# Volxel/Volxel

Hardware: AMD Instinct MI355X
Metric: Gsamples/s raymarch @512^3 vol, 1080p; achieved HBM GB/s vs peak, 1/2/4/8 GPU (higher is better)
Workload: dtype f32

## Files before the change

### include/volxel_hip.h

```cpp
#ifndef VOLXEL_HIP_H
#define VOLXEL_HIP_H

#include <stdint.h>

#ifdef __cplusplus
extern "C" {
#endif

#define VX_OK 0
#define VX_ERR_INVALID 1
#define VX_ERR_DEVICE 2
#define VX_ERR_NO_VOLUME 3
#define VX_ERR_NO_DEVICE 4

enum VxRenderMode {
  VX_MODE_DEFAULT = 0,
  VX_MODE_NO_DDA = 1,
  VX_MODE_RAYMARCH = 2,
  VX_MODE_DVR = 3,
  VX_MODE_DVR_PHONG = 4,
  VX_MODE_MIP = 5,
  VX_MODE_MINIP = 6
};

// ... 356 lines not shown
  int32_t source;
  float iso;
  uint32_t box_lo[3];
  uint32_t box_hi[3];
  uint32_t max_vertices;
  uint32_t max_triangles;
} VxMeshParams;
typedef struct VxMeshResult {
  uint64_t vertices, triangles, active_blocks, blocks;
  uint32_t bbox_lo[3], bbox_hi[3];
} VxMeshResult;
int vx_mesh_extract(VxContext* ctx, const VxMeshParams* params, VxMeshResult* out);
int vx_mesh_read(VxContext* ctx, float* verts_xyz, int32_t* cells_xyz, uint32_t* tris);
int vx_mesh_stats(VxContext* ctx, uint32_t* launches, double* kernel_ms);

int vx_debug_unorm_table(VxContext* ctx, float* out256);
int vx_debug_build_skip_mask(const uint32_t* range_packed, const uint32_t brick_count[3], const float* tf_rgba,
                             uint32_t tf_len, const VxParams* params, uint32_t* bits_out, uint32_t* level_out,
                             uint32_t dims_out[3]);
int vx_debug_build_projection_bounds(const uint32_t* range_packed, const uint32_t brick_count[3], const VxParams* params,
                                     float* bounds_out, uint32_t* level_out, uint32_t dims_out[3]);
int vx_debug_classify_miss_blocks(const VxParams* params, uint32_t width, uint32_t height, uint8_t* flags_out, uint32_t* n_out);
int vx_debug_last_launch_blocks(VxContext* ctx, uint32_t* heavy_out, uint32_t* miss_out);

#ifdef __cplusplus
}
#endif
#endif
```

### volxel_amd/_abi.py

```python
from __future__ import annotations

import ctypes as C
import os
import re

_ROOT = os.path.dirname(os.path.dirname(os.path.abspath(__file__)))
INCLUDE_DIR = os.path.join(_ROOT, "include")
LIB_PATH = os.environ.get("VOLXEL_HIP_LIB") or os.path.join(os.path.dirname(os.path.abspath(__file__)), "libvolxel_hip.so")

_CTYPES = {
    "float": C.c_float, "double": C.c_double, "int32_t": C.c_int32, "uint32_t": C.c_uint32,
    "uint64_t": C.c_uint64, "int64_t": C.c_int64,
}


def struct_from_header(header: str, name: str):
    text = open(os.path.join(INCLUDE_DIR, header)).read()
    text = re.sub(r"/\*.*?\*/", "", text, flags=re.S)
    m = re.search(r"typedef\s+struct\s+%s\s*\{(.*?)\}\s*%s\s*;" % (name, name), text, flags=re.S)
    if not m:
        raise RuntimeError(f"struct {name} not found in {header}")
    fields = []
    for decl in m.group(1).split(";"):
        decl = decl.strip()
# ... 106 lines not shown
        "vx_read_accum": ([vp, vp], i32),
        "vx_read_display": ([vp, vp, C.c_float, C.c_float], i32),
        "vx_read_display_scaled": ([vp, vp, u32, u32, C.c_float, C.c_float], i32),
        "vx_slab_info": ([vp, P(u64), P(u32)], i32),
        "vx_probe_tile_costs": ([vp, vp, u32], i32),
        "vx_set_tile_order": ([vp, vp, u32], i32),
        "vx_render_size": ([vp, P(u32), P(u32)], i32),
        "vx_slab_device_ptr": ([vp, P(vp)], i32),
        "vx_detile": ([vp, vp, vp], i32),
        "vx_get_counters": ([vp, P(VxCounters)], i32),
        "vx_reset_counters": ([vp], i32),
        "vx_device_info": ([vp, C.c_char_p, u32, P(u32), P(u64)], i32),
        "vx_version": ([], C.c_char_p),
        "vx_debug_unorm_table": ([vp, vp], i32),
        "vx_debug_rng": ([vp, i32, vp, vp, u32, vp], i32),
        "vx_probe_gather_rate": ([vp, u32, u32, P(C.c_double), P(u32)], i32),
        "vx_probe_gather_spread": ([vp, u32, P(u64)], i32),
        "vx_probe_valu_rate": ([vp, P(C.c_double), P(u32)], i32),
        "vx_upload_stats": ([vp, P(C.c_double), P(u64), P(i32)], i32),
        "vx_debug_build_skip_mask": ([vp, P(u32), vp, u32, P(VxParams), vp, P(u32), P(u32)], i32),
        "vx_debug_build_projection_bounds": ([vp, P(u32), P(VxParams), vp, P(u32), P(u32)], i32),
        "vx_debug_classify_miss_blocks": ([P(VxParams), u32, u32, vp, P(u32)], i32),
        "vx_debug_last_launch_blocks": ([vp, P(u32), P(u32)], i32),
        "vx_shadow_stats": ([vp, P(u64), P(u64), P(C.c_double)], i32),
        "vx_debug_read_shadow_grid": ([vp, vp, P(u32)], i32),
        "vx_slice": ([vp, P(VxSliceParams), vp, vp], i32),
        "vx_slice_stats": ([vp, P(u64), P(C.c_double)], i32),
        "vx_isosurface": ([vp, P(VxIsoParams), vp, vp], i32),
        "vx_iso_stats": ([vp, P(u64), P(u64), P(u64), P(u64), P(u64), P(C.c_double)], i32),
        "vx_segment": ([vp, P(VxSegmentParams), P(VxSegmentResult)], i32),
        "vx_segment_read_mask": ([vp, vp, u64], i32),
        "vx_slice_segment_mask": ([vp, P(VxSliceParams), vp], i32),
        "vx_segment_stats": ([vp, P(u32), P(u64), P(C.c_double)], i32),
        "vx_set_segment_view": ([vp, i32], i32),
        "vx_get_segment_view": ([vp, P(i32)], i32),
        "vx_segment_edit": ([vp, P(VxSegmentEditParams), P(VxSegmentResult)], i32),
        "vx_segment_write_mask": ([vp, vp, u64, P(VxSegmentResult)], i32),
        "vx_segment_edit_stats": ([vp, P(u32), P(C.c_double)], i32),
        "vx_segment_threshold": ([vp, P(VxSegmentParams), P(VxSegmentResult)], i32),
        "vx_segment_islands": ([vp, P(VxIslandsParams), P(VxIslandsResult)], i32),
        "vx_islands_read": ([vp, u64, u64, P(VxIsland)], i32),
        "vx_islands_read_labels": ([vp, vp, u64], i32),
        "vx_islands_stats": ([vp, P(u32), P(C.c_double)], i32),
        "vx_segment_distance": ([vp, P(VxDistanceParams), P(VxDistanceResult)], i32),
        "vx_distance_read": ([vp, vp, u64], i32),
        "vx_segment_margin": ([vp, P(VxMarginParams), P(VxSegmentResult)], i32),
# ... 45 lines not shown
```

### volxel_amd/csrc/vx_api.hip

```cpp
#include <hip/hip_runtime.h>

#include <algorithm>
#include <cmath>
#include <cstdio>
#include <cstdlib>
#include <cstring>
#include <string>
#include <vector>

#include "vx_dvr.hpp"
#include "vx_dvr_lds.hpp"
#include "vx_dvr_miss.hpp"
#include "vx_kernels.hpp"
#include "vx_shadow.hpp"
#include "vx_projection.hpp"
#include "vx_context.hpp"

using namespace vx;

namespace {

thread_local std::string g_create_error;

bool dvr_miss_switch() {
  const char* v = getenv("VX_DVR_MISS");
  return !(v && atoi(v) == 0);
}
Switches read_switches() {
  Switches sw;
  if (const char* v = getenv("VX_DVR_KERNEL"); v && !strcmp(v, "generic")) sw.dvr_variant = 0;
  if (const char* v = getenv("VX_DVR_FUSE")) sw.dvr_fuse = atoi(v) != 0;
  if (const char* v = getenv("VX_RAY_SHORTCUTS"); v && atoi(v) == 0) sw.ray_shortcuts = false;
  if (const char* v = getenv("VX_AUTO_CELLQUAD_MAX_BYTES")) sw.cellquad_max_bytes = strtoull(v, nullptr, 10);
  if (const char* v = getenv("VX_SEG_CHECK_MAX")) sw.seg_check_max = (uint32_t)std::min(std::max(atoi(v), 1), 4096);
  if (const char* v = getenv("VX_DIST_LDS_BYTES")) sw.dist_lds_bytes = (uint32_t)std::min(std::max(atoi(v), 256), 65536);
  sw.dvr_miss = dvr_miss_switch();
  return sw;
}

static void drain_events(VxContext* c) {
  for (auto& e : c->pending_events) {
    (void)hipEventSynchronize(e.b);
    float ms = 0.f;
    if (hipEventElapsedTime(&ms, e.a, e.b) == hipSuccess) {
      if (e.merge) {
        c->merge_ms += ms;
      } else {
        c->kernel_ms += ms;
        c->last_kernel_ms = ms;
      }
    }
    e.merge = false;
    c->free_events.push_back(e);
  }
  c->pending_events.clear();
}

static void update_tilemap(VxContext* c) {
  TileMap& t = c->tm;
// ... 214 lines not shown

enum class Kernel {
  DVR_LDS,
  PROJ_LDS,
  DVR_CQ,
  GENERIC,
};
struct LaunchPlan {
  Kernel kernel = Kernel::GENERIC;
  int mode = VX_MODE_DVR;
  int layout = VX_LAYOUT_REFERENCE;
  bool phong = false;
  bool minip = false;
  bool shadow = false;
  bool skip = false;
  bool u8 = false;
  bool probe = false;
  ShadowGrid light{};
  const float* bounds = nullptr;
  const uint32_t* order = nullptr;
  dim3 grid, block{256};
  dim3 miss_grid{0};
  const uint32_t* miss_order = nullptr;
  size_t lds = 0;
  bool fuse = false;
  bool segv = false;
  const uint32_t* segm = nullptr;
  uint32_t seg_inv = 0u;
};

static bool tuned_possible(const VxContext* c) {
  return c->sw.dvr_variant != 0 && !c->params.debug_hits && c->tf_len <= TF_LDS_MAX &&
         (c->params.dvr_ert_tau > 0.0f || proj_mode(c->params.render_mode));
}
static bool use_lds_kernel(const VxContext* c) {
  if (!tuned_possible(c)) return false;
  if (proj_mode(c->params.render_mode))
    return eff_layout(c) == VX_LAYOUT_BRICKF32 || (eff_layout(c) == VX_LAYOUT_BRICKU8 && c->vol.dv.bu != nullptr);
  if (eff_layout(c) == VX_LAYOUT_BRICKU8)
    return (c->params.render_mode == VX_MODE_DVR || c->params.render_mode == VX_MODE_DVR_PHONG) && c->vol.dv.bu != nullptr;
  if (c->params.render_mode == VX_MODE_DVR) return eff_layout(c) == VX_LAYOUT_BRICKF32;
  return c->params.render_mode == VX_MODE_DVR_PHONG && c->vol.dv.bf != nullptr;
}
static bool is_tuned(const VxContext* c) {
  const bool dvr_cq = c->params.render_mode == VX_MODE_DVR && eff_layout(c) == VX_LAYOUT_CELLQUAD;
  return tuned_possible(c) && (dvr_cq || use_lds_kernel(c));
// ... 32 lines not shown
  if (lp.kernel == Kernel::PROJ_LDS) {
    lp.skip = p.dvr_skip_empty && c->proj_dev && !c->vol.proj_table.stale;
    lp.bounds = lp.skip ? c->proj_dev : nullptr;
  } else {
    lp.skip = p.dvr_skip_empty && c->vol.dv.skip_bits;
  }
  if (c->vol.seg_view != VX_SEGVIEW_OFF && lds_window_kernel(lp.kernel)) {
    lp.segv = true;
    lp.segm = reinterpret_cast<const uint32_t*>(c->vol.seg.seg);
    lp.seg_inv = c->vol.seg_view == VX_SEGVIEW_HIDE ? ~0u : 0u;
    lp.skip = false;
    lp.bounds = nullptr;
  }
  lp.u8 = lp.layout == VX_LAYOUT_BRICKU8 && c->vol.dv.bu;
  lp.probe = probe;
  lp.order = probe ? nullptr : c->order;
  const bool lds_window = lds_window_kernel(lp.kernel);
  lp.grid = dim3(frame_blocks(c) * (lds_window && mo.count == 0u ? 1u : mo.count));
  lp.fuse = c->sw.dvr_fuse && folds(lp.kernel, lp.mode, mo.count);
  lp.lds = lds_bytes(c, lp);
  const VxContext::MissSplit& ms = c->miss;
  if (lp.kernel == Kernel::DVR_LDS && !lp.phong && !lp.shadow && !lp.segv && mo.count > 1u && c->sw.dvr_miss && ms.proved > 0u &&
      ms.table.current(p) && ms.blocks == frame_blocks(c) && !ms.split_stale) {
    lp.grid = dim3((ms.blocks - ms.n_miss) * mo.count);
    lp.order = ms.order_heavy;
    lp.miss_grid = dim3(ms.n_miss * mo.count);
    lp.miss_order = ms.order_miss;
  }
  return lp;
}

template <class F>
static void with_mode(int m, F&& f) {
  switch (m) {
    case VX_MODE_DEFAULT: f(std::integral_constant<int, VX_MODE_DEFAULT>{}); break;
    case VX_MODE_NO_DDA: f(std::integral_constant<int, VX_MODE_NO_DDA>{}); break;
    case VX_MODE_RAYMARCH: f(std::integral_constant<int, VX_MODE_RAYMARCH>{}); break;
    case VX_MODE_DVR: f(std::integral_constant<int, VX_MODE_DVR>{}); break;
    case VX_MODE_MIP: f(std::integral_constant<int, VX_MODE_MIP>{}); break;
    case VX_MODE_MINIP: f(std::integral_constant<int, VX_MODE_MINIP>{}); break;
    default: f(std::integral_constant<int, VX_MODE_DVR_PHONG>{}); break;
  }
}

static int launch_planned(VxContext* c, const LaunchPlan& lp, const MultiOut& mo, float weight) {
  if (mo.fuse && !folds(lp.kernel, lp.mode, mo.count))
    VX_FAIL(c, VX_ERR_INVALID, "render launch: running mean to fold (MultiOut::fuse) for a kernel that does not fold it");
  const VxParams& p = c->params;
  const DevVolume& v = c->vol.dv;
  const TileMap& tm = c->tm;
  const float4* tf = c->tf;
  const uint32_t n = c->tf_len;
  const hipStream_t s = c->stream;
  switch (lp.kernel) {
    case Kernel::DVR_LDS:
      if (lp.segv) {
        with_bool(lp.u8, [&](auto u8) {
          with_bool(lp.phong, [&](auto ph) {
            constexpr bool PH = decltype(ph)::value;
            hipLaunchKernelGGL((render_dvr_lds_seg<(PH ? VX_LDS_S_PHONG : VX_LDS_S), PH, decltype(u8)::value>), lp.grid, lp.block,
                               lp.lds, s, p, v, tf, n, mo, weight, tm, lp.order, lp.segm, lp.seg_inv);
          });
        });
        break;
      }
      if (lp.miss_grid.x != 0u)
        hipLaunchKernelGGL(render_dvr_miss, lp.miss_grid, lp.block, mo.fuse ? 4u * 320u * sizeof(float) : 0u, s, p, v, tf, n, mo,
                           weight, tm, lp.miss_order);
      if (lp.grid.x == 0u) break;
      with_bool(lp.skip, [&](auto sk) {
        with_bool(lp.u8, [&](auto u8) {
          constexpr bool SK = decltype(sk)::value, U8 = decltype(u8)::value;
          if (lp.shadow) {
            hipLaunchKernelGGL((render_dvr_lds_shadow<VX_LDS_S, SK, U8>), lp.grid, lp.block, lp.lds, s, p, v, tf, n, mo, weight, tm,
                               lp.order, lp.light);
            return;
          }
          with_bool(lp.phong, [&](auto ph) {
            constexpr bool PH = decltype(ph)::value;
            hipLaunchKernelGGL((render_dvr_lds<(PH ? VX_LDS_S_PHONG : VX_LDS_S), PH, SK, U8>), lp.grid, lp.block, lp.lds, s, p, v, tf,
                               n, mo, weight, tm, lp.order);
          });
        });
      });
      break;
    case Kernel::PROJ_LDS:
      if (lp.segv) {
        with_bool(lp.minip, [&](auto mi) {
          with_bool(lp.u8, [&](auto u8) {
            hipLaunchKernelGGL((render_proj_lds_seg<VX_LDS_S, decltype(mi)::value, decltype(u8)::value>), lp.grid, lp.block, lp.lds, s,
                               p, v, tf, n, mo, weight, tm, lp.order, lp.segm, lp.seg_inv);
// ... 14 lines not shown
      with_bool(lp.skip, [&](auto sk) {
        with_bool(lp.probe, [&](auto pr) {
          hipLaunchKernelGGL((render_dvr_cq<4, decltype(sk)::value, decltype(pr)::value>), lp.grid, lp.block, lp.lds, s, p, v, tf, n,
                             mo, weight, tm, lp.order);
        });
      });
      break;
    default:
      with_layout(lp.layout, [&](auto lay) {
        constexpr int LAY = decltype(lay)::value;
        if (lp.shadow) {
          hipLaunchKernelGGL((render_generic_shadow<LAY>), lp.grid, lp.block, lp.lds, s, p, v, tf, n, mo, weight, tm, lp.light);
          return;
        }
        with_mode(lp.mode, [&](auto m) {
          hipLaunchKernelGGL((render_generic<decltype(m)::value, LAY>), lp.grid, lp.block, lp.lds, s, p, v, tf, n, mo, weight, tm);
        });
      });
  }
  VX_HIP(c, hipGetLastError());
  {
    const uint32_t slots = mo.count == 0u ? 1u : mo.count;
    c->miss.last_heavy = lp.grid.x / slots;
    c->miss.last_miss = lp.miss_grid.x / slots;
  }
  return VX_OK;
}

static int set_slab_table(VxContext* c, const std::vector<const float4*>& t) {
  if (t == c->slab_table_host) return VX_OK;
  c->slab_table_host.clear();
  VX_HIP(c, hipStreamSynchronize(c->stream));
  if (int rc = c->slab_table.ensure(c, t.size())) return rc;
  VX_HIP(c, hipMemcpy(c->slab_table, t.data(), t.size() * sizeof(float4*), hipMemcpyHostToDevice));
  c->slab_table_host = t;
  return VX_OK;
}

static int launch_detile(VxContext* c, float4* image) {
  if (c->slab_table_host.size() != c->tm.shard_count)
    VX_FAIL(c, VX_ERR_INVALID, "detile: %zu slabs for %u shards", c->slab_table_host.size(), c->tm.shard_count);
  dim3 grid((c->W + 15) / 16, (c->H + 15) / 16);
  hipLaunchKernelGGL(detile, grid, dim3(256), 0, c->stream, (const float4* const*)c->slab_table, image, c->tm);
  VX_HIP(c, hipGetLastError());
  return VX_OK;
}

// ... 15 lines not shown
    if (m->W != d->W || m->H != d->H || m->tm.shard_count != t.size())
      VX_FAIL(c, VX_ERR_INVALID, "member %zu (device %d): framebuffer differs from member 0's", i, m->device);
    t[i] = m->slab;
  }
  VX_HIP(c, hipSetDevice(d->device));
  if (int rc = set_slab_table(d, t)) return member_fail(c, 0, rc);
  for (size_t i = 1; i < t.size(); ++i) {
    VxContext* m = c->members[i];
    VX_HIP(c, hipSetDevice(m->device));
    VX_HIP(c, hipEventRecord(m->done, m->stream));
  }
  VX_HIP(c, hipSetDevice(d->device));
  for (size_t i = 1; i < t.size(); ++i) VX_HIP(c, hipStreamWaitEvent(d->stream, c->members[i]->done, 0));
  return on_member0(c, launch_detile(d, d->image));
}

static int ensure_miss_split(VxContext* c) {
  VxContext::MissSplit& ms = c->miss;
  const VxParams& p = c->params;
  if (!c->sw.dvr_miss || p.render_mode != VX_MODE_DVR || !use_lds_kernel(c)) return VX_OK;
  const uint32_t nb = frame_blocks(c);
  if (!ms.table.current(p) || ms.blocks != nb) {
    ms.table.stale = true;
    std::vector<uint8_t> img;
    ms.proved = ms.n_miss = 0;
    ms.blocks = nb;
    if (classify_miss_blocks(p, c->W, c->H, img) != 0u) {
      const TileMap& tm = c->tm;
      const uint32_t nbx = (c->W + 15u) / 16u;
      auto morton_x = [](uint32_t m) { return (m & 1u) | ((m >> 1) & 2u) | ((m >> 2) & 4u); };
      ms.flags_host.assign(nb, 0);
      for (uint32_t b = 0; b < nb; ++b) {
        const uint32_t lt = (b >> 7) * 8u + (b & 7u), wt = ((b >> 3) & 15u) * 4u;
        const uint32_t pos = lt * tm.shard_count + tm.shard_rank;
        const uint32_t t = (!c->tile_perm_host.empty() && pos < tm.n_tiles) ? c->tile_perm_host[pos] : pos;
        const uint32_t x0 = (t % tm.tiles_x) * 64u + morton_x(wt) * 8u, y0 = (t / tm.tiles_x) * 64u + morton_x(wt >> 1) * 8u;
        if (lt >= tm.tiles_per_shard || t >= tm.n_tiles || x0 >= tm.W || y0 >= tm.H) {
          ms.flags_host[b] = 1;
        } else if (img[(size_t)(y0 >> 4) * nbx + (x0 >> 4)]) {
          ms.flags_host[b] = 1;
          ms.proved += 1;
        }
        ms.n_miss += ms.flags_host[b];
      }
    }
    if (ms.proved > 0u) {
      if (ms.flags.cap < nb || ms.order_heavy.cap < nb || ms.order_miss.cap < nb) {
        VX_HIP(c, hipStreamSynchronize(c->stream));
        if (int rc = ms.flags.alloc(c, nb)) return rc;
        if (int rc = ms.order_heavy.alloc(c, nb)) return rc;
        if (int rc = ms.order_miss.alloc(c, nb)) return rc;
      }
      VxContext::MissSplit::Stage& st = ms.stage[ms.next_stage];
      ms.next_stage ^= 1;
      if (st.pending) VX_HIP(c, hipEventSynchronize(st.done));
      st.pending = false;
      if (st.cap < nb) {
        if (st.p) (void)hipHostFree(st.p);
        st.p = nullptr;
        st.cap = 0;
        VX_HIP(c, hipHostMalloc(reinterpret_cast<void**>(&st.p), nb, hipHostMallocDefault));
        st.cap = nb;
      }
      if (!st.done) VX_HIP(c, hipEventCreateWithFlags(&st.done, hipEventDisableTiming));
      memcpy(st.p, ms.flags_host.data(), nb);
      VX_HIP(c, hipMemcpyAsync(ms.flags, st.p, nb, hipMemcpyHostToDevice, c->stream));
      VX_HIP(c, hipEventRecord(st.done, c->stream));
// ... 775 lines not shown
  if (!range_packed || !brick_count || !p) return VX_ERR_INVALID;
  uint32_t extent[3] = {brick_count[0] * 8u, brick_count[1] * 8u, brick_count[2] * 8u};
  std::vector<float> lohi;
  int level = 1;
  uint32_t md[3];
  compute_projection_bounds(*p, range_packed, brick_count, extent, lohi, level, md);
  if (level_out) *level_out = (uint32_t)level;
  if (dims_out) { dims_out[0] = md[0]; dims_out[1] = md[1]; dims_out[2] = md[2]; }
  if (bounds_out) memcpy(bounds_out, lohi.data(), lohi.size() * sizeof(float));
  return VX_OK;
}

int vx_debug_classify_miss_blocks(const VxParams* p, uint32_t width, uint32_t height, uint8_t* flags_out, uint32_t* n_out) {
  if (!p || width == 0 || height == 0 || width > 16384 || height > 16384) return VX_ERR_INVALID;
  std::vector<uint8_t> flags;
  uint32_t n = 0;
  if (dvr_miss_switch()) n = classify_miss_blocks(*p, width, height, flags);
  else flags.assign((size_t)((width + 15u) / 16u) * ((height + 15u) / 16u), 0);
  if (flags_out) memcpy(flags_out, flags.data(), flags.size());
  if (n_out) *n_out = n;
  return VX_OK;
}

int vx_debug_last_launch_blocks(VxContext* c, uint32_t* heavy, uint32_t* miss) {
  if (!c) return VX_ERR_INVALID;
  uint32_t h = 0, m = 0;
  for (const VxContext* k : is_group(c) ? c->members : std::vector<VxContext*>{c}) {
    h += k->miss.last_heavy;
    m += k->miss.last_miss;
  }
  if (heavy) *heavy = h;
  if (miss) *miss = m;
  return VX_OK;
}

int vx_debug_rng(VxContext* c, int op, const uint32_t* a, const uint32_t* b, uint32_t n, uint32_t* out) {
  if (!c || !a || !out || n == 0 || n > 65536u || op < 0 || op > 4 || (op == 0 && !b)) return VX_ERR_INVALID;
  if (is_group(c)) return on_member0(c, vx_debug_rng(c->members[0], op, a, b, n, out));
  VX_DEV(c);
  const uint32_t n_in = op < 2 ? n : 1u;
  uint32_t *da = nullptr, *db = nullptr, *dout = nullptr;
  hipError_t e = hipMalloc(&da, (size_t)n_in * 4);
  if (e == hipSuccess) e = hipMalloc(&db, (size_t)n_in * 4);
  if (e == hipSuccess) e = hipMalloc(&dout, (size_t)n * 4);
  if (e == hipSuccess) e = hipMemcpyAsync(da, a, (size_t)n_in * 4, hipMemcpyHostToDevice, c->stream);
  if (e == hipSuccess && op == 0) e = hipMemcpyAsync(db, b, (size_t)n_in * 4, hipMemcpyHostToDevice, c->stream);
// ... 160 lines not shown
```

### volxel_amd/csrc/vx_context.hpp

```cpp
#pragma once

#include <array>
#include <cmath>
#include <cstdint>
#include <cstdio>
#include <cstring>
#include <optional>
#include <string>
#include <type_traits>
#include <vector>

#include "vx_host.hpp"
#include "vx_types.hpp"

namespace vx __attribute__((visibility("hidden"))) {

struct EventPair {
  hipEvent_t a, b;
  bool merge = false;
};

struct Switches {
  int dvr_variant = -1;
  bool dvr_fuse = true;
  bool ray_shortcuts = true;
  std::optional<uint64_t> cellquad_max_bytes;
  uint32_t seg_check_max = 64;
  bool dvr_miss = true;
  uint32_t dist_lds_bytes = 65536;
};


template <class... T>
std::array<uint32_t, (sizeof(T) + ...) / 4> key_of(const T&... v) {
  static_assert(((sizeof(T) % 4 == 0) && ...), "key fields are 4-byte values");
  std::array<uint32_t, (sizeof(T) + ...) / 4> k{};
  uint32_t* o = k.data();
  ((memcpy(o, &v, sizeof v), o += sizeof v / 4), ...);
  return k;
}
inline auto skip_key(const VxParams& p) { return key_of(p.volume_density_scale, p.volume_inv_maj, p.sample_range); }
inline auto proj_key(const VxParams& p) { return key_of(p.volume_density_scale, p.volume_inv_maj, p.render_mode); }
inline auto iso_key(const VxParams& p) { return key_of(p.volume_density_scale, p.volume_inv_maj); }
inline auto lmaj_key(const VxParams& p) { return key_of(p.volume_density_scale, p.volume_inv_maj, p.volume_maj, p.sample_range); }
inline auto shadow_key(const VxParams& p) {
  return key_of(p.light_dir, p.density_transform_inv, p.volume_aabb_min, p.volume_aabb_max, p.volume_maj, p.volume_inv_maj,
                p.volume_density_scale, p.sample_range, p.dvr_step_voxels, p.dvr_ert_tau, p.dvr_max_steps, p.dvr_shadow_stride);
}
inline auto miss_key(const VxParams& p) {
  return key_of(p.camera_view_inv, p.camera_proj_inv, p.camera_ortho, p.volume_aabb_min, p.volume_aabb_max, p.res, p.shard_rank,
                p.shard_count);
}

template <auto KEY>
struct DerivedTable {
  bool stale = true;
  decltype(KEY(VxParams{})) key{};
  bool current(const VxParams& p) const { return !stale && KEY(p) == key; }
  void built(const VxParams& p) {
    key = KEY(p);
    stale = false;
  }
};

}

using namespace vx;

struct VxContext : VxCore {
  hipStream_t own_stream = nullptr;
  hipDeviceProp_t prop;

  struct Volume {
    bool has_volume = false;
// ... 62 lines not shown
  VxParams params{};
  bool has_params = false;

  uint32_t W = 0, H = 0;
  TileMap tm{};
  DevBuf<float4> slab;
  size_t slab_quads = 0;
  DevBuf<float4> image;
  DevBuf<float4> env_tex;
  DevBuf<float> env_imp;
  DevBuf<float4> env_impq;
  float env_avg_w = 0.0f;
  uint32_t env_w = 0, env_h = 0;
  DevBuf<uchar4> display;
  DevBuf<uint32_t> tile_perm;
  uint32_t tile_perm_n = 0;
  std::vector<uint32_t> tile_perm_host;
  struct MissSplit {
    DerivedTable<miss_key> table;
    std::vector<uint8_t> flags_host;
    DevBuf<uint8_t> flags;
    DevBuf<uint32_t> order_heavy, order_miss;
    uint32_t blocks = 0;
    uint32_t n_miss = 0, proved = 0;
    bool split_stale = true;
    uint32_t last_heavy = 0, last_miss = 0;
    struct Stage {
      uint8_t* p = nullptr;
      size_t cap = 0;
      hipEvent_t done = nullptr;
      bool pending = false;
    } stage[2];
    int next_stage = 0;
    MissSplit() = default;
    MissSplit(const MissSplit&) = delete;
    MissSplit& operator=(const MissSplit&) = delete;
    ~MissSplit() {
      for (Stage& st : stage) {
        if (st.p) (void)hipHostFree(st.p);
        if (st.done) (void)hipEventDestroy(st.done);
      }
    }
  } miss;

  DevBuf<DevCounters> dc;
  size_t dc_waves = 0;
  DevBuf<uint32_t> order;
  int tex_checked_res[2] = {-1, -1};
  bool tex_by_reciprocal[2] = {false, false};
// ... 177 lines not shown
```

### volxel_amd/csrc/vx_dvr_miss.hpp

```cpp
#pragma once
#include "vx_dvr_lds.hpp"

namespace vx {

VXD V3 dvr_miss_dir(const VxParams& p, const DevVolume& v, int px, int py, uint32_t frame) {
  float tex_x = tex_coord(px, p.res[0], &v, 0);
  float tex_y = tex_coord(py, p.res[1], &v, 1);
  float jx = 0.5f, jy = 0.5f;
  if (p.dvr_jitter) {
    Rng s = seed_xoshiro(tea32(42u * (uint32_t)(py * p.res[0] + px), frame));
    float a0 = rng(s), a1 = rng(s), b0 = rng(s), b1 = rng(s);
    jx = (a0 + b0) / 2.0f;
    jy = (a1 + b1) / 2.0f;
  }
  return setup_world_ray(p, tex_x, tex_y, jx, jy, &v).d;
}

__global__ __launch_bounds__(256) __attribute__((amdgpu_waves_per_eu(8, 8))) void render_dvr_miss(
    const VxParams p, const DevVolume v, const float4* __restrict__ tf_global, uint32_t tf_len, const MultiOut mo, float weight,
    const TileMap tm, const uint32_t* __restrict__ order) {
  extern __shared__ float fold_lds[];
  uint32_t fslot, bslot;
  multi_slot(blockIdx.x, mo.count, fslot, bslot);
  const uint32_t blk = order[bslot];
// ... 8 lines not shown
  if (mo.count > 1u) {
    uint32_t base;
    const uint32_t sh = fuse ? frame_group<6>(fslot, mo.count, base) : frame_group<VX_DVR_FL_MAXSH>(fslot, mo.count, base);
    if (sh != 0u) {
      const uint32_t psh = 6u - sh;
      plane = ((fslot - base) << psh) + (lane & ((1u << psh) - 1u));
      slab = lane_frame_slot(base + (lane >> psh), my_frame);
    }
  }
  int px, py;
  uint32_t si;
  const bool in_image = wave_pixel(tm, lt, wt, plane, px, py, si);
  DvrRay r{};
  if (in_image) r.wdir = dvr_miss_dir(p, v, px, py, my_frame);
  if (fuse != 0u) {
    V3 L = v3(0.f, 0.f, 0.f);
    if (in_image) L = dvr_radiance(p, v, r, 0.0f, 0.0f, 0.0f, 1.0f);
    fold_frames(fold_lds + (threadIdx.x >> 6) * 320u, lane, L, in_image, si, mo.accum, fuse, 31u - (uint32_t)__builtin_clz(mo.count));
  } else if (in_image) dvr_store(p, v, r, 0.0f, 0.0f, 0.0f, 1.0f, weight, slab, si);
  const uint32_t n_px = (uint32_t)__builtin_popcountll(ballot(in_image));
  add_counts(dc, 0u, 0u, n_px, 0u, 0u, 0u, blk);
}

__global__ __launch_bounds__(1024) void split_order(const uint32_t* __restrict__ order, const uint8_t* __restrict__ miss, uint32_t n,
                                                     uint32_t* __restrict__ heavy, uint32_t* __restrict__ light) {
  __shared__ uint32_t cnt[1024];
  const uint32_t per = (n + 1023u) / 1024u;
  const uint32_t lo = min(threadIdx.x * per, n), hi = min(lo + per, n);
  auto is_miss = [&](uint32_t b) { return b < n && miss[b] != 0; };
  uint32_t m = 0;
  for (uint32_t i = lo; i < hi; ++i) m += is_miss(order[i]) ? 1u : 0u;
  cnt[threadIdx.x] = m;
  __syncthreads();
  for (uint32_t off = 1; off < 1024u; off <<= 1) {
    const uint32_t add = threadIdx.x >= off ? cnt[threadIdx.x - off] : 0u;
    __syncthreads();
    cnt[threadIdx.x] += add;
    __syncthreads();
  }
  uint32_t mpos = cnt[threadIdx.x] - m, hpos = lo - mpos;
  for (uint32_t i = lo; i < hi; ++i) {
    const uint32_t b = order[i];
    if (is_miss(b)) light[mpos++] = b;
    else heavy[hpos++] = b;
  }
}

}
```

### volxel_amd/csrc/vx_host.hpp

```cpp
#pragma once
#include <hip/hip_runtime.h>

#include <algorithm>
#include <cmath>
#include <cstdint>
#include <cstdio>
#include <cstring>
#include <string>
#include <type_traits>
#include <utility>
#include <vector>

#include "../../include/volxel_hip.h"


struct VxCore {
  int device = 0;
  hipStream_t stream = nullptr;
  std::string err;
};

#define VX_FAIL(ctx, code, ...)                       \
  do {                                                \
    char buf_[512];                                   \
// ... 40 lines not shown
  int ensure(VxCore* c, size_t n) { return n > cap ? alloc(c, n) : VX_OK; }
};

struct Carve {
  uintptr_t base = 0;
  size_t off = 0;
  template <class T>
  T* take(size_t n = 1) {
    T* r = base ? reinterpret_cast<T*>(base + off) : nullptr;
    off += n * sizeof(T);
    return r;
  }
};
template <class F>
int carve(VxCore* c, DevBuf<void>& buf, F&& layout) {
  Carve measure;
  layout(measure);
  if (int rc = buf.alloc(c, measure.off)) return rc;
  Carve k{reinterpret_cast<uintptr_t>(buf.p)};
  layout(k);
  return VX_OK;
}

inline uint32_t classify_miss_blocks(const VxParams& p, uint32_t W, uint32_t H, std::vector<uint8_t>& flags) {
  const uint32_t nbx = (W + 15u) / 16u, nby = (H + 15u) / 16u;
  flags.assign((size_t)nbx * nby, 0);
  if (p.camera_ortho || W == 0 || H == 0) return 0;
  const float* vi = p.camera_view_inv;
  const float* pi = p.camera_proj_inv;
  for (int i = 0; i < 16; ++i)
    if (!std::isfinite(vi[i]) || !std::isfinite(pi[i])) return 0;
  for (int i = 0; i < 3; ++i)
    if (!std::isfinite(p.volume_aabb_min[i]) || !std::isfinite(p.volume_aabb_max[i]) || !(p.volume_aabb_min[i] <= p.volume_aabb_max[i]))
      return 0;
  if (vi[3] != 0.0f || vi[7] != 0.0f || vi[11] != 0.0f || vi[15] != 1.0f) return 0;
  if (pi[3] != 0.0f || pi[7] != 0.0f || pi[15] == 0.0f) return 0;
  const double s = pi[15] > 0.0f ? 1.0 : -1.0;
  double B[3][3];
  for (int r = 0; r < 3; ++r) {
    const int cols[3] = {0, 4, 12};
    for (int k = 0; k < 3; ++k)
      B[r][k] = (double)vi[r] * pi[cols[k]] + (double)vi[4 + r] * pi[cols[k] + 1] + (double)vi[8 + r] * pi[cols[k] + 2];
  }
  const double c00 = B[1][1] * B[2][2] - B[1][2] * B[2][1], c01 = B[1][2] * B[2][0] - B[1][0] * B[2][2],
               c02 = B[1][0] * B[2][1] - B[1][1] * B[2][0];
  const double det = B[0][0] * c00 + B[0][1] * c01 + B[0][2] * c02;
  double scale = 0.0;
  for (auto& row : B)
    for (double x : row) scale = std::max(scale, std::fabs(x));
  if (!std::isfinite(det) || !(std::fabs(det) > 1e-12 * scale * scale * scale)) return 0;
  const double Bi[3][3] = {
      {c00 / det, (B[0][2] * B[2][1] - B[0][1] * B[2][2]) / det, (B[0][1] * B[1][2] - B[0][2] * B[1][1]) / det},
      {c01 / det, (B[0][0] * B[2][2] - B[0][2] * B[2][0]) / det, (B[0][2] * B[1][0] - B[0][0] * B[1][2]) / det},
      {c02 / det, (B[0][1] * B[2][0] - B[0][0] * B[2][1]) / det, (B[0][0] * B[1][1] - B[0][1] * B[1][0]) / det}};
  const double cam[3] = {vi[12], vi[13], vi[14]};
  bool inside = true;
  double diag2 = 0.0;
  for (int i = 0; i < 3; ++i) {
    inside = inside && cam[i] >= p.volume_aabb_min[i] && cam[i] <= p.volume_aabb_max[i];
    const double e = (double)p.volume_aabb_max[i] - p.volume_aabb_min[i];
    diag2 += e * e;
  }
  if (inside) return 0;
  const double axis_len = std::sqrt(B[0][2] * B[0][2] + B[1][2] * B[1][2] + B[2][2] * B[2][2]);
  const double margin = 1e-4 * std::sqrt(diag2) + 1e-9;
  double pt[8][2];
// ... 34 lines not shown
  for (int k = 0; k < na; ++k) {
    double lo = 1e300, hi = -1e300;
    for (int i = 0; i < 8; ++i) {
      const double t = axes[k].nx * pt[i][0] + axes[k].ny * pt[i][1];
      lo = std::min(lo, t);
      hi = std::max(hi, t);
    }
    axes[k].lo = lo;
    axes[k].hi = hi;
  }
  constexpr double GAP = 2.0;
  uint32_t n = 0;
  for (uint32_t by = 0; by < nby; ++by)
    for (uint32_t bx = 0; bx < nbx; ++bx) {
      const double x0 = 16.0 * bx + 0.5, x1 = 16.0 * bx + 15.5, y0 = 16.0 * by + 0.5, y1 = 16.0 * by + 15.5;
      bool separated = false;
      for (int k = 0; k < na && !separated; ++k) {
        const double ax = axes[k].nx, ay = axes[k].ny;
        const double rlo = std::min(ax * x0, ax * x1) + std::min(ay * y0, ay * y1);
        const double rhi = std::max(ax * x0, ax * x1) + std::max(ay * y0, ay * y1);
        separated = rlo - axes[k].hi >= GAP || axes[k].lo - rhi >= GAP;
      }
      if (separated) {
        flags[(size_t)by * nbx + bx] = 1;
        ++n;
      }
    }
  return n;
}

inline float f16_bits_to_float(uint16_t h) {
  _Float16 v;
  memcpy(&v, &h, 2);
  return (float)v;
}
inline int skip_level_for(const uint32_t extent[3]) {
  for (int g = 1; g <= 3; ++g) {
    uint64_t n = 1;
    for (int a = 0; a < 3; ++a) n *= (uint64_t)(extent[a] >> (3 + g)) + 1u;
    if (n <= 65536u) return g;
  }
  return 3;
}
inline void compute_skip_mask(const VxParams& p, const uint32_t* range_packed, const uint32_t bc[3],
                              const uint32_t extent[3], const float* tf_rgba, uint32_t L,
                              std::vector<uint32_t>& bits, int& level_out, uint32_t md[3]) {
// ... 151 lines not shown
```

### volxel_amd/renderer.py

```python
from __future__ import annotations

import ctypes as C
import math

import numpy as np

from . import _abi
from .scene import Camera, Grid, Volume, flat, from_flat
from .environment import Environment
from .settings import ViewerSettings, verify_settings
from .transfer import default_transfer_function, generate_transfer_function
from ._errors import VolxelError
from .renderer_mesh import MeshMixin
from .renderer_segment import (Histogram, IslandSegment, Islands, Segment, SegmentComparison, SegmentDistance,
                               SegmentMixin)
from .renderer_view import ViewMixin

LOW_RESOLUTION_DURATION = 5


def sample_weight(frame_index: int, low_res_duration: int = LOW_RESOLUTION_DURATION) -> float:
    if frame_index < low_res_duration:
        return 0.0
    return (frame_index - low_res_duration) / (frame_index - low_res_duration + 1)
# ... 435 lines not shown
                    "timePerSample": total / self.frame_index, "totalTime": total,
                    "viewport": [0, 0, rf * self.canvas_width, rf * self.canvas_height],
                    "device": device,
                    "timestamp": datetime.datetime.now(datetime.timezone.utc).isoformat().replace("+00:00", "Z"),
                })
        finally:
            self.low_res_preview = saved_preview
            if not saved_preview:
                self.resolution_factor = 1.0
                self._resize_framebuffers_to_canvas()
        return results

    def counters(self):
        c = _abi.VxCounters()
        self._check(self._lib.vx_get_counters(self._ctx, C.byref(c)))
        return c

    def reset_counters(self):
        self._check(self._lib.vx_reset_counters(self._ctx))

    def last_launch_blocks(self):
        return self._out("vx_debug_last_launch_blocks", C.c_uint32, C.c_uint32)

    def set_stream(self, hip_stream: int | None):
        self._check(self._lib.vx_set_stream(self._ctx, C.c_void_p(hip_stream or 0)))

    def set_layout(self, layout: int):
        self._check(self._lib.vx_set_layout(self._ctx, int(layout)))

    def upload_stats(self):
        s, b, pin = self._out("vx_upload_stats", C.c_double, C.c_uint64, C.c_int)
        return s, b, bool(pin)

    def shadow_stats(self):
        return self._out("vx_shadow_stats", C.c_uint64, C.c_uint64, C.c_double)

    def read_shadow_grid(self) -> np.ndarray:
        dims = (C.c_uint32 * 3)()
        self._check(self._lib.vx_debug_read_shadow_grid(self._ctx, None, dims))
        out = np.empty((dims[2], dims[1], dims[0]), dtype=np.float32)
        self._check(self._lib.vx_debug_read_shadow_grid(self._ctx, out.ctypes.data, dims))
        return out

    def probe_gather_rate(self, lines: int, distinct: int | None = None):
        d = int(lines) if distinct is None else int(distinct)
        return self._out("vx_probe_gather_rate", C.c_double, C.c_uint32, args=(int(lines), d))
# ... 49 lines not shown
```

Baseline: 1094.

## Add constant-background kernel for miss blocks whose environment color is provably constant

Adds a host-side classifier that proves which screen blocks see a constant sky colour, either because the environment is hidden or because the view cone stays away from the light-direction highlight. Those miss blocks go to a new lightweight kernel that writes the precomputed colour, skipping per-pixel environment evaluation. split_order now partitions blocks three ways, and the miss-table key gains light and environment parameters. The proof leans on the highlight term (pow 300 with a 0.9 cutoff) underflowing so the colour stays exact, and a debug kernel checks that assumption exhaustively.

```diff
diff --git a/include/volxel_hip.h b/include/volxel_hip.h
--- a/include/volxel_hip.h
+++ b/include/volxel_hip.h
@@ -402,6 +402,10 @@
                                      float* bounds_out, uint32_t* level_out, uint32_t dims_out[3]);
 int vx_debug_classify_miss_blocks(const VxParams* params, uint32_t width, uint32_t height, uint8_t* flags_out, uint32_t* n_out);
 int vx_debug_last_launch_blocks(VxContext* ctx, uint32_t* heavy_out, uint32_t* miss_out);
+int vx_debug_classify_const_background_blocks(const VxParams* params, uint32_t width, uint32_t height, uint8_t* flags_out,
+                                              uint32_t* n_out);
+int vx_debug_last_launch_const_blocks(VxContext* ctx, uint32_t* const_out);
+int vx_debug_const_background_mismatches(VxContext* ctx, uint64_t* count_out);
 
 #ifdef __cplusplus
 }
diff --git a/volxel_amd/_abi.py b/volxel_amd/_abi.py
--- a/volxel_amd/_abi.py
+++ b/volxel_amd/_abi.py
@@ -152,6 +152,9 @@
         "vx_debug_build_projection_bounds": ([vp, P(u32), P(VxParams), vp, P(u32), P(u32)], i32),
         "vx_debug_classify_miss_blocks": ([P(VxParams), u32, u32, vp, P(u32)], i32),
         "vx_debug_last_launch_blocks": ([vp, P(u32), P(u32)], i32),
+        "vx_debug_classify_const_background_blocks": ([P(VxParams), u32, u32, vp, P(u32)], i32),
+        "vx_debug_last_launch_const_blocks": ([vp, P(u32)], i32),
+        "vx_debug_const_background_mismatches": ([vp, P(u64)], i32),
         "vx_shadow_stats": ([vp, P(u64), P(u64), P(C.c_double)], i32),
         "vx_debug_read_shadow_grid": ([vp, vp, P(u32)], i32),
         "vx_slice": ([vp, P(VxSliceParams), vp, vp], i32),
diff --git a/volxel_amd/csrc/vx_api.hip b/volxel_amd/csrc/vx_api.hip
--- a/volxel_amd/csrc/vx_api.hip
+++ b/volxel_amd/csrc/vx_api.hip
@@ -25,6 +25,10 @@
 bool dvr_miss_switch() {
   const char* v = getenv("VX_DVR_MISS");
   return !(v && atoi(v) == 0);
+}
+bool dvr_const_switch() {
+  const char* v = getenv("VX_DVR_CONST");
+  return dvr_miss_switch() && !(v && atoi(v) == 0);
 }
 Switches read_switches() {
   Switches sw;
@@ -35,6 +39,7 @@
   if (const char* v = getenv("VX_SEG_CHECK_MAX")) sw.seg_check_max = (uint32_t)std::min(std::max(atoi(v), 1), 4096);
   if (const char* v = getenv("VX_DIST_LDS_BYTES")) sw.dist_lds_bytes = (uint32_t)std::min(std::max(atoi(v), 256), 65536);
   sw.dvr_miss = dvr_miss_switch();
+  sw.dvr_const = dvr_const_switch();
   return sw;
 }
 
@@ -295,6 +300,8 @@
   dim3 grid, block{256};
   dim3 miss_grid{0};
   const uint32_t* miss_order = nullptr;
+  dim3 const_grid{0};
+  const uint32_t* const_order = nullptr;
   size_t lds = 0;
   bool fuse = false;
   bool segv = false;
@@ -373,10 +380,13 @@
   const VxContext::MissSplit& ms = c->miss;
   if (lp.kernel == Kernel::DVR_LDS && !lp.phong && !lp.shadow && !lp.segv && mo.count > 1u && c->sw.dvr_miss && ms.proved > 0u &&
       ms.table.current(p) && ms.blocks == frame_blocks(c) && !ms.split_stale) {
+    const uint32_t n_const = lp.fuse ? ms.n_const : 0u;
     lp.grid = dim3((ms.blocks - ms.n_miss) * mo.count);
     lp.order = ms.order_heavy;
-    lp.miss_grid = dim3(ms.n_miss * mo.count);
+    lp.miss_grid = dim3((ms.n_miss - n_const) * mo.count);
     lp.miss_order = ms.order_miss;
+    lp.const_grid = dim3(n_const);
+    lp.const_order = ms.order_miss + (ms.n_miss - n_const);
   }
   return lp;
 }
@@ -418,6 +428,8 @@
       if (lp.miss_grid.x != 0u)
         hipLaunchKernelGGL(render_dvr_miss, lp.miss_grid, lp.block, mo.fuse ? 4u * 320u * sizeof(float) : 0u, s, p, v, tf, n, mo,
                            weight, tm, lp.miss_order);
+      if (lp.const_grid.x != 0u)
+        hipLaunchKernelGGL(render_dvr_const, lp.const_grid, lp.block, 0, s, p, v, tf, n, mo, weight, tm, lp.const_order);
       if (lp.grid.x == 0u) break;
       with_bool(lp.skip, [&](auto sk) {
         with_bool(lp.u8, [&](auto u8) {
@@ -478,7 +490,8 @@
   {
     const uint32_t slots = mo.count == 0u ? 1u : mo.count;
     c->miss.last_heavy = lp.grid.x / slots;
-    c->miss.last_miss = lp.miss_grid.x / slots;
+    c->miss.last_miss = lp.miss_grid.x / slots + lp.const_grid.x;
+    c->miss.last_const = lp.const_grid.x;
   }
   return VX_OK;
 }
@@ -540,10 +553,12 @@
   const uint32_t nb = frame_blocks(c);
   if (!ms.table.current(p) || ms.blocks != nb) {
     ms.table.stale = true;
-    std::vector<uint8_t> img;
-    ms.proved = ms.n_miss = 0;
+    std::vector<uint8_t> img, same;
+    ms.proved = ms.n_miss = ms.n_const = 0;
     ms.blocks = nb;
     if (classify_miss_blocks(p, c->W, c->H, img) != 0u) {
+      if (c->sw.dvr_const) classify_const_background_blocks(p, c->W, c->H, same);
+      else same.assign(img.size(), 0);
       const TileMap& tm = c->tm;
       const uint32_t nbx = (c->W + 15u) / 16u;
       auto morton_x = [](uint32_t m) { return (m & 1u) | ((m >> 1) & 2u) | ((m >> 2) & 4u); };
@@ -554,13 +569,20 @@
         const uint32_t t = (!c->tile_perm_host.empty() && pos < tm.n_tiles) ? c->tile_perm_host[pos] : pos;
         const uint32_t x0 = (t % tm.tiles_x) * 64u + morton_x(wt) * 8u, y0 = (t / tm.tiles_x) * 64u + morton_x(wt >> 1) * 8u;
         if (lt >= tm.tiles_per_shard || t >= tm.n_tiles || x0 >= tm.W || y0 >= tm.H) {
-          ms.flags_host[b] = 1;
+          ms.flags_host[b] = 3;
         } else if (img[(size_t)(y0 >> 4) * nbx + (x0 >> 4)]) {
-          ms.flags_host[b] = 1;
+          ms.flags_host[b] = same[(size_t)(y0 >> 4) * nbx + (x0 >> 4)] ? 2 : 1;
           ms.proved += 1;
+          ms.n_const += ms.flags_host[b] == 2;
         }
-        ms.n_miss += ms.flags_host[b];
+        ms.n_miss += ms.flags_host[b] != 0;
       }
+      const uint8_t empty_kind = ms.n_const > 0u ? 2 : 1;
+      for (uint32_t b = 0; b < nb; ++b)
+        if (ms.flags_host[b] == 3) {
+          ms.flags_host[b] = empty_kind;
+          ms.n_const += empty_kind == 2;
+        }
     }
     if (ms.proved > 0u) {
       if (ms.flags.cap < nb || ms.order_heavy.cap < nb || ms.order_miss.cap < nb) {
@@ -1382,6 +1404,44 @@
   return VX_OK;
 }
 
+int vx_debug_classify_const_background_blocks(const VxParams* p, uint32_t width, uint32_t height, uint8_t* flags_out, uint32_t* n_out) {
+  if (!p || width == 0 || height == 0 || width > 16384 || height > 16384) return VX_ERR_INVALID;
+  std::vector<uint8_t> flags;
+  uint32_t n = 0;
+  if (dvr_const_switch()) n = classify_const_background_blocks(*p, width, height, flags);
+  else flags.assign((size_t)((width + 15u) / 16u) * ((height + 15u) / 16u), 0);
+  if (flags_out) memcpy(flags_out, flags.data(), flags.size());
+  if (n_out) *n_out = n;
+  return VX_OK;
+}
+
+int vx_debug_last_launch_const_blocks(VxContext* c, uint32_t* const_out) {
+  if (!c) return VX_ERR_INVALID;
+  uint32_t n = 0;
+  for (const VxContext* k : is_group(c) ? c->members : std::vector<VxContext*>{c}) n += k->miss.last_const;
+  if (const_out) *const_out = n;
+  return VX_OK;
+}
+
+int vx_debug_const_background_mismatches(VxContext* c, uint64_t* count_out) {
+  if (!c || !count_out) return VX_ERR_INVALID;
+  if (is_group(c)) return on_member0(c, vx_debug_const_background_mismatches(c->members[0], count_out));
+  VX_DEV(c);
+  DevBuf<unsigned long long> bad;
+  if (int rc = bad.alloc(c, 1)) return rc;
+  uint32_t last_bits;
+  const float c0 = CONST_BACKGROUND_C0;
+  memcpy(&last_bits, &c0, 4);
+  VX_HIP(c, hipMemsetAsync(bad, 0, sizeof(unsigned long long), c->stream));
+  hipLaunchKernelGGL(count_const_background_mismatches, dim3(16384), dim3(256), 0, c->stream, last_bits, bad);
+  VX_HIP(c, hipGetLastError());
+  unsigned long long n = 0;
+  VX_HIP(c, hipMemcpyAsync(&n, bad, sizeof n, hipMemcpyDeviceToHost, c->stream));
+  VX_HIP(c, hipStreamSynchronize(c->stream));
+  *count_out = n;
+  return VX_OK;
+}
+
 int vx_debug_last_launch_blocks(VxContext* c, uint32_t* heavy, uint32_t* miss) {
   if (!c) return VX_ERR_INVALID;
   uint32_t h = 0, m = 0;
diff --git a/volxel_amd/csrc/vx_context.hpp b/volxel_amd/csrc/vx_context.hpp
--- a/volxel_amd/csrc/vx_context.hpp
+++ b/volxel_amd/csrc/vx_context.hpp
@@ -27,6 +27,7 @@
   std::optional<uint64_t> cellquad_max_bytes;
   uint32_t seg_check_max = 64;
   bool dvr_miss = true;
+  bool dvr_const = true;
   uint32_t dist_lds_bytes = 65536;
 };
 
@@ -49,7 +50,7 @@
 }
 inline auto miss_key(const VxParams& p) {
   return key_of(p.camera_view_inv, p.camera_proj_inv, p.camera_ortho, p.volume_aabb_min, p.volume_aabb_max, p.res, p.shard_rank,
-                p.shard_count);
+                p.shard_count, p.light_dir, p.use_env, p.show_environment);
 }
 
 template <auto KEY>
@@ -158,9 +159,10 @@
     DevBuf<uint8_t> flags;
     DevBuf<uint32_t> order_heavy, order_miss;
     uint32_t blocks = 0;
-    uint32_t n_miss = 0, proved = 0;
+    uint32_t n_miss = 0, n_const = 0, proved = 0;
     bool split_stale = true;
     uint32_t last_heavy = 0, last_miss = 0;
+    uint32_t last_const = 0;
     struct Stage {
       uint8_t* p = nullptr;
       size_t cap = 0;
diff --git a/volxel_amd/csrc/vx_dvr_miss.hpp b/volxel_amd/csrc/vx_dvr_miss.hpp
--- a/volxel_amd/csrc/vx_dvr_miss.hpp
+++ b/volxel_amd/csrc/vx_dvr_miss.hpp
@@ -54,28 +54,106 @@
   add_counts(dc, 0u, 0u, n_px, 0u, 0u, 0u, blk);
 }
 
-__global__ __launch_bounds__(1024) void split_order(const uint32_t* __restrict__ order, const uint8_t* __restrict__ miss, uint32_t n,
-                                                     uint32_t* __restrict__ heavy, uint32_t* __restrict__ light) {
-  __shared__ uint32_t cnt[1024];
-  const uint32_t per = (n + 1023u) / 1024u;
-  const uint32_t lo = min(threadIdx.x * per, n), hi = min(lo + per, n);
-  auto is_miss = [&](uint32_t b) { return b < n && miss[b] != 0; };
-  uint32_t m = 0;
-  for (uint32_t i = lo; i < hi; ++i) m += is_miss(order[i]) ? 1u : 0u;
-  cnt[threadIdx.x] = m;
-  __syncthreads();
-  for (uint32_t off = 1; off < 1024u; off <<= 1) {
-    const uint32_t add = threadIdx.x >= off ? cnt[threadIdx.x - off] : 0u;
-    __syncthreads();
-    cnt[threadIdx.x] += add;
-    __syncthreads();
+VXD DevCounters* lane_frame_counters(uint32_t my_fslot) {
+  struct KArgs { VxParams p; DevVolume v; const float4* tf; uint32_t tf_len; MultiOut mo; };
+  typedef const char __attribute__((address_space(4)))* KPtr;
+  const KPtr ka = (KPtr)__builtin_amdgcn_kernarg_segment_ptr() + offsetof(KArgs, mo);
+  return ((DevCounters* const __attribute__((address_space(4)))*)(ka + offsetof(MultiOut, dc)))[my_fslot];
+}
+__global__ __launch_bounds__(256) void render_dvr_const(const VxParams p, const DevVolume v, const float4* __restrict__ tf_global,
+                                                        uint32_t tf_len, const MultiOut mo, float weight, const TileMap tm,
+                                                        const uint32_t* __restrict__ order) {
+  const uint32_t blk = order[blockIdx.x];
+  uint32_t lt, sub;
+  if (!block_to_tile(blk, tm, lt, sub)) return;
+  const uint32_t wave = threadIdx.x >> 6, lane = threadIdx.x & 63u, count = mo.count;
+  int px, py;
+  uint32_t si;
+  const bool in_image = wave_pixel(tm, lt, sub * 4u + wave, lane, px, py, si);
+  float Lx = 0.0f * p.dvr_gain[0], Ly = 0.0f * p.dvr_gain[1], Lz = 0.0f * p.dvr_gain[2];
+  if (p.show_environment > 0) {
+    const float e = p.env_strength * fma_(0.0f, 4.0f, 0.01f);
+    Lx = fma_(1.0f, e, Lx);
+    Ly = fma_(1.0f, e, Ly);
+    Lz = fma_(1.0f, e, Lz);
   }
-  uint32_t mpos = cnt[threadIdx.x] - m, hpos = lo - mpos;
-  for (uint32_t i = lo; i < hi; ++i) {
-    const uint32_t b = order[i];
-    if (is_miss(b)) light[mpos++] = b;
-    else heavy[hpos++] = b;
+  const float rx = fma_(1.0f, sanitize1(Lx), 0.0f), ry = fma_(1.0f, sanitize1(Ly), 0.0f), rz = fma_(1.0f, sanitize1(Lz), 0.0f);
+  if (in_image) {
+    float4 acc = mo.accum[si];
+    if (mo.fuse == 1u) {
+      for (uint32_t k = 0; k < count; ++k) {
+        const float w = mo.weight[k], omw = 1.0f - w;
+        acc.x = fma_(omw, rx, w * acc.x);
+        acc.y = fma_(omw, ry, w * acc.y);
+        acc.z = fma_(omw, rz, w * acc.z);
+      }
+    } else {
+      for (uint32_t k = 0; k < count; ++k) {
+        const float w = mo.weight[k], omw = 1.0f - w;
+        acc.x = fma_(omw, rx, w * (w != 0.0f ? acc.x : 0.0f));
+        acc.y = fma_(omw, ry, w * (w != 0.0f ? acc.y : 0.0f));
+        acc.z = fma_(omw, rz, w * (w != 0.0f ? acc.z : 0.0f));
+      }
+    }
+    acc.w = 1.0f;
+    mo.accum[si] = acc;
+  }
+  const unsigned long long inimg = ballot(in_image);
+  if (lane < count) {
+    const uint32_t npx = 64u / count;
+    const unsigned long long mine = (inimg >> (lane * npx)) & (~0ull >> (64u - npx));
+    DevCounters* const w = lane_frame_counters(lane) + (blk * 4u + wave);
+    w->pixels += count * (uint32_t)__builtin_popcountll(mine);
+    w->last_slots = 0u;
   }
 }
 
+__global__ __launch_bounds__(1024) void split_order(const uint32_t* __restrict__ order, const uint8_t* __restrict__ kind, uint32_t n,
+                                                     uint32_t* __restrict__ heavy, uint32_t* __restrict__ light) {
+  __shared__ uint32_t cnt[2][1024];
+  const uint32_t per = (n + 1023u) / 1024u;
+  const uint32_t lo = min(threadIdx.x * per, n), hi = min(lo + per, n);
+  auto kind_of = [&](uint32_t b) { return b < n ? (uint32_t)kind[b] : 0u; };
+  uint32_t m[2] = {0u, 0u};
+  for (uint32_t i = lo; i < hi; ++i) {
+    const uint32_t k = kind_of(order[i]);
+    m[0] += k == 1u ? 1u : 0u;
+    m[1] += k >= 2u ? 1u : 0u;
+  }
+  cnt[0][threadIdx.x] = m[0];
+  cnt[1][threadIdx.x] = m[1];
+  __syncthreads();
+  for (uint32_t off = 1; off < 1024u; off <<= 1) {
+    const uint32_t add0 = threadIdx.x >= off ? cnt[0][threadIdx.x - off] : 0u;
+    const uint32_t add1 = threadIdx.x >= off ? cnt[1][threadIdx.x - off] : 0u;
+    __syncthreads();
+    cnt[0][threadIdx.x] += add0;
+    cnt[1][threadIdx.x] += add1;
+    __syncthreads();
+  }
+  uint32_t mpos = cnt[0][threadIdx.x] - m[0], cpos = cnt[1][threadIdx.x] - m[1], hpos = lo - mpos - cpos;
+  cpos += cnt[0][1023];
+  for (uint32_t i = lo; i < hi; ++i) {
+    const uint32_t b = order[i], k = kind_of(b);
+    if (k == 0u) heavy[hpos++] = b;
+    else if (k == 1u) light[mpos++] = b;
+    else light[cpos++] = b;
+  }
 }
+
+__global__ __launch_bounds__(256) void count_const_background_mismatches(uint32_t last_bits, unsigned long long* __restrict__ bad) {
+  const float want = 0.01f;
+  uint32_t n = 0;
+  auto differs = [&](uint32_t bits) {
+    const float c = gl_max(__uint_as_float(bits), 0.0f);
+    const float s = gl_clamp(powf(c, 300.0f), 0.0f, 1.0f);
+    return __float_as_uint(fma_(s, 4.0f, 0.01f)) != __float_as_uint(want) ? 1u : 0u;
+  };
+  for (unsigned long long i = (unsigned long long)blockIdx.x * 256u + threadIdx.x; i <= last_bits; i += (unsigned long long)gridDim.x * 256u)
+    n += differs((uint32_t)i);
+  if (blockIdx.x == 0u && threadIdx.x == 0u) n += differs(0x80000000u);
+  n = wave_sum(n);
+  if ((threadIdx.x & 63u) == 0u && n != 0u) atomicAdd(bad, (unsigned long long)n);
+}
+
+}
diff --git a/volxel_amd/csrc/vx_host.hpp b/volxel_amd/csrc/vx_host.hpp
--- a/volxel_amd/csrc/vx_host.hpp
+++ b/volxel_amd/csrc/vx_host.hpp
@@ -86,26 +86,38 @@
   return VX_OK;
 }
 
+struct PinholeRays {
+  double B[3][3];
+  double s;
+};
+inline bool pinhole_rays(const VxParams& p, PinholeRays& r) {
+  if (p.camera_ortho) return false;
+  const float* vi = p.camera_view_inv;
+  const float* pi = p.camera_proj_inv;
+  for (int i = 0; i < 16; ++i)
+    if (!std::isfinite(vi[i]) || !std::isfinite(pi[i])) return false;
+  if (vi[3] != 0.0f || vi[7] != 0.0f || vi[11] != 0.0f || vi[15] != 1.0f) return false;
+  if (pi[3] != 0.0f || pi[7] != 0.0f || pi[15] == 0.0f) return false;
+  r.s = pi[15] > 0.0f ? 1.0 : -1.0;
+  for (int row = 0; row < 3; ++row) {
+    const int cols[3] = {0, 4, 12};
+    for (int k = 0; k < 3; ++k)
+      r.B[row][k] = (double)vi[row] * pi[cols[k]] + (double)vi[4 + row] * pi[cols[k] + 1] + (double)vi[8 + row] * pi[cols[k] + 2];
+  }
+  return true;
+}
+
 inline uint32_t classify_miss_blocks(const VxParams& p, uint32_t W, uint32_t H, std::vector<uint8_t>& flags) {
   const uint32_t nbx = (W + 15u) / 16u, nby = (H + 15u) / 16u;
   flags.assign((size_t)nbx * nby, 0);
-  if (p.camera_ortho || W == 0 || H == 0) return 0;
+  PinholeRays rays;
+  if (W == 0 || H == 0 || !pinhole_rays(p, rays)) return 0;
   const float* vi = p.camera_view_inv;
-  const float* pi = p.camera_proj_inv;
-  for (int i = 0; i < 16; ++i)
-    if (!std::isfinite(vi[i]) || !std::isfinite(pi[i])) return 0;
   for (int i = 0; i < 3; ++i)
     if (!std::isfinite(p.volume_aabb_min[i]) || !std::isfinite(p.volume_aabb_max[i]) || !(p.volume_aabb_min[i] <= p.volume_aabb_max[i]))
       return 0;
-  if (vi[3] != 0.0f || vi[7] != 0.0f || vi[11] != 0.0f || vi[15] != 1.0f) return 0;
-  if (pi[3] != 0.0f || pi[7] != 0.0f || pi[15] == 0.0f) return 0;
-  const double s = pi[15] > 0.0f ? 1.0 : -1.0;
-  double B[3][3];
-  for (int r = 0; r < 3; ++r) {
-    const int cols[3] = {0, 4, 12};
-    for (int k = 0; k < 3; ++k)
-      B[r][k] = (double)vi[r] * pi[cols[k]] + (double)vi[4 + r] * pi[cols[k] + 1] + (double)vi[8 + r] * pi[cols[k] + 2];
-  }
+  const double s = rays.s;
+  const auto& B = rays.B;
   const double c00 = B[1][1] * B[2][2] - B[1][2] * B[2][1], c01 = B[1][2] * B[2][0] - B[1][0] * B[2][2],
                c02 = B[1][0] * B[2][1] - B[1][1] * B[2][0];
   const double det = B[0][0] * c00 + B[0][1] * c01 + B[0][2] * c02;
@@ -186,6 +198,53 @@
         separated = rlo - axes[k].hi >= GAP || axes[k].lo - rhi >= GAP;
       }
       if (separated) {
+        flags[(size_t)by * nbx + bx] = 1;
+        ++n;
+      }
+    }
+  return n;
+}
+
+constexpr float CONST_BACKGROUND_C0 = 0.9f;
+inline uint32_t classify_const_background_blocks(const VxParams& p, uint32_t W, uint32_t H, std::vector<uint8_t>& flags) {
+  const uint32_t nbx = (W + 15u) / 16u, nby = (H + 15u) / 16u;
+  flags.assign((size_t)nbx * nby, 0);
+  PinholeRays rays;
+  if (W == 0 || H == 0 || !pinhole_rays(p, rays)) return 0;
+  if (p.show_environment <= 0) {
+    std::fill(flags.begin(), flags.end(), (uint8_t)1);
+    return (uint32_t)flags.size();
+  }
+  if (p.use_env != 0) return 0;
+  const double nl[3] = {-(double)p.light_dir[0], -(double)p.light_dir[1], -(double)p.light_dir[2]};
+  const double light_len = std::sqrt(nl[0] * nl[0] + nl[1] * nl[1] + nl[2] * nl[2]);
+  if (!std::isfinite(light_len)) return 0;
+  auto dir = [&](double X, double Y, double d[3]) {
+    const double nx = 2.0 * X / (double)W - 1.0, ny = 2.0 * Y / (double)H - 1.0;
+    for (int i = 0; i < 3; ++i) d[i] = rays.s * (rays.B[i][0] * nx + rays.B[i][1] * ny + rays.B[i][2]);
+  };
+  auto angle = [](const double a[3], const double b[3]) {
+    const double cx = a[1] * b[2] - a[2] * b[1], cy = a[2] * b[0] - a[0] * b[2], cz = a[0] * b[1] - a[1] * b[0];
+    return std::atan2(std::sqrt(cx * cx + cy * cy + cz * cz), a[0] * b[0] + a[1] * b[1] + a[2] * b[2]);
+  };
+  constexpr double GAP = 2.0;
+  const double limit = (double)CONST_BACKGROUND_C0 - 1e-3;
+  uint32_t n = 0;
+  for (uint32_t by = 0; by < nby; ++by)
+    for (uint32_t bx = 0; bx < nbx; ++bx) {
+      const double x0 = 16.0 * bx + 0.5 - GAP, x1 = 16.0 * bx + 15.5 + GAP, y0 = 16.0 * by + 0.5 - GAP, y1 = 16.0 * by + 15.5 + GAP;
+      double dc[3], d[3], rho = 0.0;
+      dir(0.5 * (x0 + x1), 0.5 * (y0 + y1), dc);
+      if (!(dc[0] * dc[0] + dc[1] * dc[1] + dc[2] * dc[2] > 0.0)) continue;
+      bool cone = true;
+      for (int corner = 0; corner < 4; ++corner) {
+        dir(corner & 1 ? x1 : x0, corner & 2 ? y1 : y0, d);
+        cone = cone && d[0] * d[0] + d[1] * d[1] + d[2] * d[2] > 0.0;
+        rho = std::max(rho, angle(dc, d));
+      }
+      if (!cone || !(rho < 1.5)) continue;
+      const double bound = light_len * std::cos(std::max(0.0, angle(dc, nl) - rho));
+      if (bound < limit) {
         flags[(size_t)by * nbx + bx] = 1;
         ++n;
       }
diff --git a/volxel_amd/renderer.py b/volxel_amd/renderer.py
--- a/volxel_amd/renderer.py
+++ b/volxel_amd/renderer.py
@@ -481,6 +481,12 @@
     def last_launch_blocks(self):
         return self._out("vx_debug_last_launch_blocks", C.c_uint32, C.c_uint32)
 
+    def last_launch_const_blocks(self):
+        return self._out("vx_debug_last_launch_const_blocks", C.c_uint32)[0]
+
+    def const_background_mismatches(self):
+        return self._out("vx_debug_const_background_mismatches", C.c_uint64)[0]
+
     def set_stream(self, hip_stream: int | None):
         self._check(self._lib.vx_set_stream(self._ctx, C.c_void_p(hip_stream or 0)))
 
```

Result: no change. 1094 (median of 4 runs) (+0.0%).
